# dannys4/MrHyDE

Hardware: AMD Instinct MI355X
Metric: assembled elements/sec (vol Jacobian+residual) (higher is better)
Workload: dtype f64; 1 GPU; 3D thermal Q2 hex, 64^3 structured mesh per GPU (affine), quadrature 4, volume Jacobian+residual assembled into CRS; elements_per_gpu=262144, dofs_per_gpu=2146689, nnz_per_gpu=135005697, partition=single block, affine_elements=262144, block_patterns=27, row_blocks=35562, row_owner_kind=1

## Files before the change

mrhyde_amd/csrc/kernels/row_gather.hip:

```cpp
#include <hip/hip_runtime.h>

#include <algorithm>

#include "device_math.hpp"
#include "launch.hpp"

namespace mha {
namespace {

__device__ __forceinline__ void wave_lds_sync() {
  __builtin_amdgcn_fence(__ATOMIC_RELEASE, "wavefront");
  __builtin_amdgcn_wave_barrier();
  __builtin_amdgcn_fence(__ATOMIC_ACQUIRE, "wavefront");
}

template <typename SlotT, int LPR, bool DOF>
__global__ __launch_bounds__(256) void row_gather_kernel(BlockDev b, RowGatherDev g, const double *__restrict__ local_J,
                                                         const double *__restrict__ local_res, double *res, double *vals,
                                                         int overwrite) {
  extern __shared__ double acc_all[];
  constexpr int RPW = 64 / LPR;
  const int wave = threadIdx.x >> 6, sub = (threadIdx.x & 63) / LPR, lane = threadIdx.x & (LPR - 1), n = b.n;
  double *acc = acc_all + (size_t)(wave * RPW + sub) * g.max_row;
  const SlotT *slot = static_cast<const SlotT *>(g.slot);
  const int nwaves = gridDim.x * 4 * RPW;
  for (int k = lane; k < g.max_row; k += LPR) acc[k] = 0.0;
  wave_lds_sync();
  struct Meta { int lo, len, i0, ni, fixed; };
  auto load_meta = [&](int row) {
    Meta m = {0, 0, 0, 0, 1};
    if (row < b.nrows) {
      m.lo = b.rowptr[row];
      m.len = b.rowptr[row + 1] - m.lo;
      m.i0 = g.inc_ptr[row];
      m.ni = g.inc_ptr[row + 1] - m.i0;
      m.fixed = (b.fixed && b.fixed[row]) ? 1 : 0;
    }
    return m;
  };
  const int row0 = (blockIdx.x * 4 + wave) * RPW + sub;
  Meta m_cur = load_meta(row0), m_nxt = load_meta(row0 + nwaves);
  int e_cur = (lane < m_cur.ni) ? g.inc_elem[m_cur.i0 + lane] : 0, p_cur = (lane < m_cur.ni) ? g.inc_pos[m_cur.i0 + lane] : 0;
  int d_cur = (DOF && lane < m_cur.ni) ? g.inc_dof[m_cur.i0 + lane] : 0;
  for (int row = row0; row < b.nrows; row += nwaves) {
    const int e_nxt = (lane < m_nxt.ni) ? g.inc_elem[m_nxt.i0 + lane] : 0;
    const int p_nxt = (lane < m_nxt.ni) ? g.inc_pos[m_nxt.i0 + lane] : 0;
    const int d_nxt = (DOF && lane < m_nxt.ni) ? g.inc_dof[m_nxt.i0 + lane] : 0;
    const Meta m_nn = load_meta(row + 2 * nwaves);
    const int lo = m_cur.lo, len = m_cur.len, i0 = m_cur.i0, ni = m_cur.ni;
    if (m_cur.fixed) {
      if (overwrite) {
        if (vals) for (int k = lane; k < len; k += LPR) vals[lo + k] = 0.0;
        if (res && lane == 0) res[row] = 0.0;
      }
    } else {
      if (vals) {
        const int total = ni * n;
        for (int t0 = 0; t0 < total; t0 += LPR) {
          const int t = t0 + lane;
          const bool valid = t < total;
          const int k = valid ? t / n : 0, sj = t - k * n;
          int e = __shfl(e_cur, k & (LPR - 1), LPR), pos = __shfl(p_cur, k & (LPR - 1), LPR);
          int dof = DOF ? __shfl(d_cur, k & (LPR - 1), LPR) : 0;
          if (valid) {
            if (k >= LPR) { e = g.inc_elem[i0 + k]; pos = g.inc_pos[i0 + k]; if constexpr (DOF) dof = g.inc_dof[i0 + k]; }
            const size_t off = ((size_t)e * n + pos) * n + sj, offd = ((size_t)e * n + pos) * n + pos;
            if constexpr (DOF) {
              const size_t so = ((size_t)e * n + pos) * n + b.offsets[sj];
              unsafeAtomicAdd(acc + slot[so], local_J[((size_t)e * n + dof) * n + sj]);
            } else {
              unsafeAtomicAdd(acc + slot[g.lump_mass ? offd : off], local_J[g.adjoint ? offd : off]);
            }
          }
        }
        wave_lds_sync();
        for (int k = lane; k < len; k += LPR) {
          const double a = acc[k];
          acc[k] = 0.0;
          vals[lo + k] = overwrite ? a : vals[lo + k] + a;
        }
        wave_lds_sync();
      }
      if (res) {
        double r = 0.0;
        for (int k = lane; k < ni; k += LPR) {
          const int e = k < LPR ? e_cur : g.inc_elem[i0 + k], pos = k < LPR ? p_cur : g.inc_pos[i0 + k];
          const int dof = !DOF ? 0 : k < LPR ? d_cur : g.inc_dof[i0 + k];
          r += local_res[(size_t)e * n + (DOF ? dof : pos)];
        }
#pragma unroll
        for (int o = LPR / 2; o > 0; o >>= 1) r += __shfl_xor(r, o, LPR);
        if (lane == 0) res[row] = overwrite ? r : res[row] + r;
      }
    }
    m_cur = m_nxt;
    m_nxt = m_nn;
    e_cur = e_nxt;
    p_cur = p_nxt;
    d_cur = d_nxt;
  }
}

}

void launch_row_gather(const BlockDev &b, const RowGatherDev &g, const double *local_J, const double *local_res,
                       double *res, double *vals, int overwrite, hipStream_t stream) {
  if (b.nrows <= 0) return;
  const bool small_rows = g.max_row <= 32 && b.n <= 16;
  const bool tiny_ok = small_rows && g.max_row <= 16 && b.n <= 8 && g.slot_bytes == 1;
  const bool medium = !small_rows && g.max_row <= 64 && b.n <= 32 && g.slot_bytes == 1 && g.inc_dof == nullptr;
  const int lpr = medium ? 16 : !small_rows ? 64 : tiny_ok ? 8 : 16;
  const int rpw = 64 / lpr;
  const size_t lds = sizeof(double) * 4 * rpw * (size_t)g.max_row;
  MHA_REQUIRE(lds <= 64 * 1024, MHA_ERR_INVALID, "CRS rows of " << g.max_row << " entries do not fit the row-gather kernel");
  const int grid = std::min((b.nrows + 4 * rpw - 1) / (4 * rpw), 256 * 8);
  auto go = [&](auto kern) {
    hipLaunchKernelGGL(kern, dim3(grid), dim3(256), lds, stream, b, g, local_J, local_res, res, vals, overwrite);
  };
  const bool dof = g.inc_dof != nullptr;
  MHA_REQUIRE(!dof || (small_rows && g.slot_bytes == 1 && !g.adjoint && !g.lump_mass), MHA_ERR_INVALID,
              "dof-ordered element arrays are gathered by the short-row kernels only");
  if (lpr == 8) { if (dof) go(row_gather_kernel<uint8_t, 8, true>); else go(row_gather_kernel<uint8_t, 8, false>); }
  else if (medium) go(row_gather_kernel<uint8_t, 16, false>);
  else if (g.slot_bytes == 1) {
    if (!small_rows) go(row_gather_kernel<uint8_t, 64, false>);
    else if (dof) go(row_gather_kernel<uint8_t, 16, true>);
    else go(row_gather_kernel<uint8_t, 16, false>);
  } else { if (small_rows) go(row_gather_kernel<uint16_t, 16, false>); else go(row_gather_kernel<uint16_t, 64, false>); }
  MHA_HIP(hipGetLastError());
}

}
```

Measured before the change: 1.440 billion elements/s.

## Restructure row-gather walk to batch slot/value loads before LDS atomics

```diff
diff --git a/mrhyde_amd/csrc/kernels/row_gather.hip b/mrhyde_amd/csrc/kernels/row_gather.hip
--- a/mrhyde_amd/csrc/kernels/row_gather.hip
+++ b/mrhyde_amd/csrc/kernels/row_gather.hip
@@ -4,6 +4,7 @@
 
 #include "device_math.hpp"
 #include "launch.hpp"
+#include "row_gather_walk.hpp"
 
 namespace mha {
 namespace {
@@ -20,34 +21,106 @@
                                                          int overwrite) {
   extern __shared__ double acc_all[];
   constexpr int RPW = 64 / LPR;
+  constexpr int D = row_walk_depth(LPR);
   const int wave = threadIdx.x >> 6, sub = (threadIdx.x & 63) / LPR, lane = threadIdx.x & (LPR - 1), n = b.n;
+  const int P = row_walk_passes(n, LPR);
+  int offs0 = 0, offs1 = 0;
+  if constexpr (DOF) {
+    offs0 = lane < n ? b.offsets[lane] : 0;
+    offs1 = lane + LPR < n ? b.offsets[lane + LPR] : 0;
+  }
+  auto group_read = [](int v, int k) {
+    if constexpr (LPR == 64) return __builtin_amdgcn_readlane(v, k);
+    else return __shfl(v, k, LPR);
+  };
   double *acc = acc_all + (size_t)(wave * RPW + sub) * g.max_row;
   const SlotT *slot = static_cast<const SlotT *>(g.slot);
   const int nwaves = gridDim.x * 4 * RPW;
   for (int k = lane; k < g.max_row; k += LPR) acc[k] = 0.0;
   wave_lds_sync();
-  struct Meta { int lo, len, i0, ni, fixed; };
+  struct Meta {
+    int lo, hi, i0, i1, fixed;
+    __device__ int len() const { return hi - lo; }
+    __device__ int ni() const { return i1 - i0; }
+  };
   auto load_meta = [&](int row) {
     Meta m = {0, 0, 0, 0, 1};
     if (row < b.nrows) {
       m.lo = b.rowptr[row];
-      m.len = b.rowptr[row + 1] - m.lo;
+      m.hi = b.rowptr[row + 1];
       m.i0 = g.inc_ptr[row];
-      m.ni = g.inc_ptr[row + 1] - m.i0;
-      m.fixed = (b.fixed && b.fixed[row]) ? 1 : 0;
+      m.i1 = g.inc_ptr[row + 1];
+      m.fixed = b.fixed ? b.fixed[row] : 0;
     }
     return m;
   };
   const int row0 = (blockIdx.x * 4 + wave) * RPW + sub;
   Meta m_cur = load_meta(row0), m_nxt = load_meta(row0 + nwaves);
-  int e_cur = (lane < m_cur.ni) ? g.inc_elem[m_cur.i0 + lane] : 0, p_cur = (lane < m_cur.ni) ? g.inc_pos[m_cur.i0 + lane] : 0;
-  int d_cur = (DOF && lane < m_cur.ni) ? g.inc_dof[m_cur.i0 + lane] : 0;
+  int e_cur = (lane < m_cur.ni()) ? g.inc_elem[m_cur.i0 + lane] : 0, p_cur = (lane < m_cur.ni()) ? g.inc_pos[m_cur.i0 + lane] : 0;
+  int d_cur = (DOF && lane < m_cur.ni()) ? g.inc_dof[m_cur.i0 + lane] : 0;
   for (int row = row0; row < b.nrows; row += nwaves) {
-    const int e_nxt = (lane < m_nxt.ni) ? g.inc_elem[m_nxt.i0 + lane] : 0;
-    const int p_nxt = (lane < m_nxt.ni) ? g.inc_pos[m_nxt.i0 + lane] : 0;
-    const int d_nxt = (DOF && lane < m_nxt.ni) ? g.inc_dof[m_nxt.i0 + lane] : 0;
+    int lo = m_cur.lo, len = m_cur.len(), i0 = m_cur.i0, ni = m_cur.ni();
+    if constexpr (LPR == 64) {
+      lo = __builtin_amdgcn_readfirstlane(lo);
+      len = __builtin_amdgcn_readfirstlane(len);
+      i0 = __builtin_amdgcn_readfirstlane(i0);
+      ni = __builtin_amdgcn_readfirstlane(ni);
+    }
+    {
+      if (vals && !m_cur.fixed) {
+        if (ni <= LPR) {
+          RowWalk w;
+          while (w.more(ni)) {
+            double v[D];
+            int s[D];
+            bool ok[D];
+#pragma unroll
+            for (int j = 0; j < D; ++j) {
+              const int sj = w.column(lane, LPR);
+              ok[j] = w.valid(lane, LPR, ni, n);
+              const int e = group_read(e_cur, w.k & (LPR - 1)), pos = group_read(p_cur, w.k & (LPR - 1));
+              const size_t rb = ((size_t)e * n + pos) * n;
+              size_t so, vo;
+              if constexpr (DOF) {
+                const int dof = group_read(d_cur, w.k & (LPR - 1));
+                so = rb + (w.p == 0 ? offs0 : offs1);
+                vo = ((size_t)e * n + dof) * n + sj;
+              } else {
+                so = rb + (g.lump_mass ? pos : sj);
+                vo = rb + (g.adjoint ? pos : sj);
+              }
+              s[j] = 0;
+              v[j] = 0.0;
+              if (ok[j]) {
+                s[j] = slot[so];
+                v[j] = local_J[vo];
+              }
+              w.advance(P);
+            }
+#pragma unroll
+            for (int j = 0; j < D; ++j)
+              if (ok[j]) unsafeAtomicAdd(acc + s[j], v[j]);
+          }
+        } else {
+          for (int k = 0; k < ni; ++k) {
+            const int e = g.inc_elem[i0 + k], pos = g.inc_pos[i0 + k];
+            const size_t rb = ((size_t)e * n + pos) * n;
+            for (int sj = lane; sj < n; sj += LPR) {
+              if constexpr (DOF) {
+                const int dof = g.inc_dof[i0 + k];
+                unsafeAtomicAdd(acc + slot[rb + b.offsets[sj]], local_J[((size_t)e * n + dof) * n + sj]);
+              } else {
+                unsafeAtomicAdd(acc + slot[rb + (g.lump_mass ? pos : sj)], local_J[rb + (g.adjoint ? pos : sj)]);
+              }
+            }
+          }
+        }
+      }
+    }
+    const int e_nxt = (lane < m_nxt.ni()) ? g.inc_elem[m_nxt.i0 + lane] : 0;
+    const int p_nxt = (lane < m_nxt.ni()) ? g.inc_pos[m_nxt.i0 + lane] : 0;
+    const int d_nxt = (DOF && lane < m_nxt.ni()) ? g.inc_dof[m_nxt.i0 + lane] : 0;
     const Meta m_nn = load_meta(row + 2 * nwaves);
-    const int lo = m_cur.lo, len = m_cur.len, i0 = m_cur.i0, ni = m_cur.ni;
     if (m_cur.fixed) {
       if (overwrite) {
         if (vals) for (int k = lane; k < len; k += LPR) vals[lo + k] = 0.0;
@@ -55,24 +128,6 @@
       }
     } else {
       if (vals) {
-        const int total = ni * n;
-        for (int t0 = 0; t0 < total; t0 += LPR) {
-          const int t = t0 + lane;
-          const bool valid = t < total;
-          const int k = valid ? t / n : 0, sj = t - k * n;
-          int e = __shfl(e_cur, k & (LPR - 1), LPR), pos = __shfl(p_cur, k & (LPR - 1), LPR);
-          int dof = DOF ? __shfl(d_cur, k & (LPR - 1), LPR) : 0;
-          if (valid) {
-            if (k >= LPR) { e = g.inc_elem[i0 + k]; pos = g.inc_pos[i0 + k]; if constexpr (DOF) dof = g.inc_dof[i0 + k]; }
-            const size_t off = ((size_t)e * n + pos) * n + sj, offd = ((size_t)e * n + pos) * n + pos;
-            if constexpr (DOF) {
-              const size_t so = ((size_t)e * n + pos) * n + b.offsets[sj];
-              unsafeAtomicAdd(acc + slot[so], local_J[((size_t)e * n + dof) * n + sj]);
-            } else {
-              unsafeAtomicAdd(acc + slot[g.lump_mass ? offd : off], local_J[g.adjoint ? offd : off]);
-            }
-          }
-        }
         wave_lds_sync();
         for (int k = lane; k < len; k += LPR) {
           const double a = acc[k];
@@ -113,7 +168,7 @@
   const int rpw = 64 / lpr;
   const size_t lds = sizeof(double) * 4 * rpw * (size_t)g.max_row;
   MHA_REQUIRE(lds <= 64 * 1024, MHA_ERR_INVALID, "CRS rows of " << g.max_row << " entries do not fit the row-gather kernel");
-  const int grid = std::min((b.nrows + 4 * rpw - 1) / (4 * rpw), 256 * 8);
+  const int grid = std::min((b.nrows + 4 * rpw - 1) / (4 * rpw), 256 * 256);
   auto go = [&](auto kern) {
     hipLaunchKernelGGL(kern, dim3(grid), dim3(256), lds, stream, b, g, local_J, local_res, res, vals, overwrite);
   };
diff --git a/mrhyde_amd/csrc/kernels/row_gather_walk.hpp b/mrhyde_amd/csrc/kernels/row_gather_walk.hpp
--- /dev/null
+++ b/mrhyde_amd/csrc/kernels/row_gather_walk.hpp
@@ -0,0 +1,30 @@
+#pragma once
+
+#if defined(__HIPCC__)
+#define MHA_WALK_HD __host__ __device__ inline
+#else
+#define MHA_WALK_HD inline
+#endif
+
+namespace mha {
+
+MHA_WALK_HD constexpr int row_walk_depth(int lpr) { return lpr == 64 ? 8 : 4; }
+
+MHA_WALK_HD constexpr int row_walk_passes(int n, int lpr) { return (n + lpr - 1) / lpr; }
+
+MHA_WALK_HD constexpr int row_walk_trips(int ni, int passes, int depth) { return (ni * passes + depth - 1) / depth; }
+
+struct RowWalk {
+  int k = 0, p = 0;
+  MHA_WALK_HD int column(int lane, int lpr) const { return lane + p * lpr; }
+  MHA_WALK_HD bool valid(int lane, int lpr, int ni, int n) const { return k < ni && column(lane, lpr) < n; }
+  MHA_WALK_HD void advance(int passes) {
+    if (++p == passes) {
+      p = 0;
+      ++k;
+    }
+  }
+  MHA_WALK_HD bool more(int ni) const { return k < ni; }
+};
+
+}
```

Result: no change. 1.437 billion elements/s (-0.2%).
